# ManUtdMoon/Distributional-Reachability-Policy-Optimization

Measured on AMD Instinct MI355X. Metric: imagined transitions/sec + SAC grad-steps/sec, quadrotor @1/2/4/8 GPU, higher is better.
Workload: dtype fp32

## Files before the change

### distributional-reachability-policy-optimization_amd/csrc/wgrad.hip

```cpp
#include "common.hpp"
#include "ens_nll.hpp"
#include "pack_layout.hpp"

using namespace drpo;

namespace {
constexpr int WG_NW = 4;
constexpr int WG_NT = WG_NW * 64;
constexpr int WG_D = 3;
constexpr int WG_ROWQ = 64;
constexpr int WG_MAXITEMS = 16;
constexpr int WG_SLD = 264;
}

#ifdef DRPO_STAMPS
__device__ unsigned long long g_stamps_wg[1 << 14][8];
#define STAMPG(i)                                                                                 \
  do {                                                                                            \
    __builtin_amdgcn_sched_barrier(0);                                                            \
    unsigned long long _t;                                                                        \
    asm volatile("s_memtime %0\n\ts_waitcnt lgkmcnt(0)" : "=s"(_t)::"memory");                    \
    __builtin_amdgcn_sched_barrier(0);                                                            \
    if (threadIdx.x == 0 && blockIdx.x < (1u << 14)) g_stamps_wg[blockIdx.x][(i)] = _t;           \
  } while (0)
DRPO_API int drpo_debug_stamps_wgrad(unsigned long long* dst, int n) {
  return (int)hipMemcpyFromSymbol(dst, HIP_SYMBOL(g_stamps_wg), sizeof(unsigned long long) * 8 * (size_t)n);
}
DRPO_API int drpo_debug_stamps_wgrad_clear() {
  void* p = nullptr;
  if (hipGetSymbolAddress(&p, HIP_SYMBOL(g_stamps_wg)) != hipSuccess) return 1;
  return (int)hipMemset(p, 0, sizeof(g_stamps_wg));
}
#else
#define STAMPG(i) \
  do {            \
  } while (0)
#endif

struct WgradPlan {
  int to, ti;
  int nto, nti, nch;
  int chunk;
  int va, vb;
  int z2;
  int pk_layer;
  int pk_z0;
  int vf;
  int64_t first_unit;
  int64_t first_tile;
  int64_t slab_off;
};

constexpr int WG_MAXSUMS = 4;

struct WgradArgs {
  int64_t first[WG_MAXITEMS];
  drpo_wgrad_item_t it[WG_MAXITEMS];
  WgradPlan pl[WG_MAXITEMS];
  int64_t units;
  int n;
  int has_red;
  drpo_ens_reduce_t red;
  int nsums;
  drpo_sum_t sums[WG_MAXSUMS];
  int has_adam;
  drpo_wgrad_adam_t adam;
  float* slab;
  unsigned* ctr;
};

typedef const __attribute__((address_space(4))) WgradArgs WgradArgsK;

__device__ __forceinline__ void sums_block(WgradArgsK& a, float* red) {
  for (int q = 0; q < a.nsums; ++q) {
    const auto& S = a.sums[q];
    float v = 0.f;
    for (int j = threadIdx.x; j < S.n; j += WG_NT) v += S.part[j];
    v = block_tree_sum(v, red);
    if (threadIdx.x == 0) *S.out = v;
    __syncthreads();
  }
}

__device__ __forceinline__ void st_sc1(float* p, float v) {
  __hip_atomic_store(p, v, __ATOMIC_RELAXED, __HIP_MEMORY_SCOPE_AGENT);
}
__device__ __forceinline__ float ld_sc1(const float* p) {
  return __hip_atomic_load(const_cast<float*>(p), __ATOMIC_RELAXED, __HIP_MEMORY_SCOPE_AGENT);
}

template <int W, bool VEC>
__device__ __forceinline__ f32x4 frag_load(const float* __restrict__ M, int64_t row, int64_t ld, int c, int ncols) {
  const float* p = M + row * ld + c;
  f32x4 v;
  if constexpr (W == 4 && VEC) {
    v = gload(reinterpret_cast<const f32x4*>(p));
  } else if constexpr (W == 4) {
#pragma unroll
    for (int u = 0; u < 4; ++u) v[u] = gload(c + u < ncols ? p + u : p);
  } else {
    v = f32x4{gload(p), 0.f, 0.f, 0.f};
  }
  return v;
}

template <int TO, int TI>
__device__ __forceinline__ void frag_mma(const f32x4& a, const f32x4& b, f32x4 (&acc)[TO / 16][TI / 16]) {
  constexpr int MA = TO / 16, MB = TI / 16;
  if constexpr (MA == 4 && MB == 4) {
#pragma unroll
    for (int m = 0; m < 4; ++m)
#pragma unroll
      for (int n = 0; n < 4; ++n) acc[m][n] = __builtin_amdgcn_mfma_f32_16x16x4f32(a[m], b[n], acc[m][n], 0, 0, 0);
  } else if constexpr (MA == 4) {
#pragma unroll
    for (int m = 0; m < 4; ++m) acc[m][0] = __builtin_amdgcn_mfma_f32_16x16x4f32(a[m], b[0], acc[m][0], 0, 0, 0);
  } else if constexpr (MB == 4) {
#pragma unroll
    for (int n = 0; n < 4; ++n) acc[0][n] = __builtin_amdgcn_mfma_f32_16x16x4f32(a[0], b[n], acc[0][n], 0, 0, 0);
  } else {
    acc[0][0] = __builtin_amdgcn_mfma_f32_16x16x4f32(a[0], b[0], acc[0][0], 0, 0, 0);
  }
}

template <int TO, int TI>
__device__ __forceinline__ int slab_index(int w, int ol, int il) {
  constexpr int NA = (TO / 16) * (TI / 16), NB = TI / 16;
  int m, rr, G, n, L;
  if constexpr (TO == 64) {
    m = ol & 3; rr = (ol >> 2) & 3; G = ol >> 4;
  } else {
    m = 0; rr = ol & 3; G = ol >> 2;
  }
  if constexpr (TI == 64) {
    n = il & 3; L = il >> 2;
  } else {
    n = 0; L = il;
  }
  return (w * NA + m * NB + n) * WG_SLD + rr * 64 + 16 * G + L;
}

__device__ __forceinline__ float wg_block_sum(float v, float* red) {
  v = wave_sum(v);
  const int lane = threadIdx.x & 63, w = threadIdx.x >> 6;
  __syncthreads();
  if (lane == 0) red[w] = v;
  __syncthreads();
  float s = 0.f;
  if (threadIdx.x == 0)
    for (int i = 0; i < WG_NW; ++i) s += red[i];
  return s;
}

struct WgUnit {
  int zb, ch;
  int o0, i0;
  int dout, din;
  int64_t tile_local;
  int64_t r0, r1;
  bool do_bias;
  bool bias_mine;
  float *gW, *gb;
  int64_t eW, eb;
};

template <int TO, int TI>
__device__ __forceinline__ WgUnit unit_decode(WgradArgsK& a, int q, int64_t u) {
  const auto& I = a.it[q];
  const auto& P = a.pl[q];
  WgUnit U;
  const unsigned uu = (unsigned)u;
  const int it_i = (int)(uu % (unsigned)P.nti);
  unsigned rest = uu / (unsigned)P.nti;
  const int it_o = (int)(rest % (unsigned)P.nto);
  rest /= (unsigned)P.nto;
  U.ch = (int)(rest % (unsigned)P.nch);
  U.zb = (int)(rest / (unsigned)P.nch);
  U.tile_local = ((int64_t)U.zb * P.nto + it_o) * P.nti + it_i;
  U.dout = I.dout;
  U.din = I.din;
  U.o0 = it_o * TO;
  U.i0 = it_i * TI;
  U.r0 = (int64_t)U.ch * P.chunk;
  U.r1 = min(I.rows, U.r0 + P.chunk);
  U.do_bias = it_i == 0;
  U.bias_mine = U.do_bias && (int)threadIdx.x < TO && U.o0 + (int)threadIdx.x < U.dout;
  U.gW = I.gW + (size_t)U.zb * I.gwstride;
  U.gb = I.gb + (size_t)U.zb * I.gbstride;
  U.eW = a.has_adam ? U.gW - a.adam.g : 0;
  U.eb = a.has_adam ? U.gb - a.adam.g : 0;
  return U;
}

template <int TO, int TI, bool VA, bool VB, bool Z2>
__device__ __forceinline__ void wgrad_accumulate(WgradArgsK& a, int q, const WgUnit& U,
                                                 f32x4 (&acc)[TO / 16][TI / 16], f32x4& bsum) {
  constexpr int MA = TO / 16, MB = TI / 16;
  constexpr int WA = TO == 64 ? 4 : 1, WB = TI == 64 ? 4 : 1;
  const auto& I = a.it[q];
  const auto& P = a.pl[q];
  const int lane = threadIdx.x & 63, wave = threadIdx.x >> 6;
  const int g = lane >> 4, l15 = lane & 15;
  const int dout = U.dout, din = U.din;
  const float* __restrict__ dz = I.dz + (size_t)U.zb * I.zstride;
  const float* __restrict__ dz2 = Z2 ? I.dz2 + (size_t)U.zb * I.zstride : nullptr;
  const float* __restrict__ y = I.y + (size_t)U.zb * I.ystride;
  const int64_t r1 = U.r1;
  const bool do_bias = U.do_bias;

  const int ca_raw = U.o0 + (WA == 4 ? 4 * l15 : l15);
  const int cb_raw = U.i0 + (WB == 4 ? 4 * l15 : l15);
  const int ca = ca_raw < dout ? ca_raw : 0, cb = cb_raw < din ? cb_raw : 0;

#pragma unroll
  for (int m = 0; m < MA; ++m)
#pragma unroll
    for (int n = 0; n < MB; ++n) acc[m][n] = f32x4{0.f, 0.f, 0.f, 0.f};
  bsum = f32x4{0.f, 0.f, 0.f, 0.f};

  const int nj = P.chunk / (4 * WG_NW);
  const int64_t rlane = U.r0 + 4 * wave + g;
  auto ld = [&](int j, f32x4& fa, f32x4& fb, f32x4& fa2) {
    const int64_t r = rlane + 16 * (int64_t)j;
    const int64_t rc = r < r1 ? r : r1 - 1;
    fa = frag_load<WA, VA>(dz, rc, dout, ca, dout);
    fb = frag_load<WB, VB>(y, rc, din, cb, din);
    if constexpr (Z2) fa2 = frag_load<WA, VA>(dz2, rc, dout, ca, dout);
  };
  auto use = [&](int j, f32x4 fa, const f32x4& fb, const f32x4& fa2) {
    if constexpr (Z2) fa += fa2;
    if (rlane + 16 * (int64_t)j >= r1) fa = f32x4{0.f, 0.f, 0.f, 0.f};
    frag_mma<TO, TI>(fa, fb, acc);
    if (do_bias) bsum += fa;
  };
  f32x4 ra[WG_D], rb[WG_D], ra2[Z2 ? WG_D : 1];
#pragma unroll
  for (int v = 0; v < WG_D; ++v) ra[v] = rb[v] = f32x4{0.f, 0.f, 0.f, 0.f};
#pragma unroll
  for (int v = 0; v < (Z2 ? WG_D : 1); ++v) ra2[v] = f32x4{0.f, 0.f, 0.f, 0.f};
  const int steps = (nj + WG_D - 1 + WG_D - 1) / WG_D * WG_D;
  STAMPG(6);
  for (int s0 = 0; s0 < steps; s0 += WG_D) {
#pragma unroll
    for (int v = 0; v < WG_D; ++v) {
      ld(s0 + v, ra[v], rb[v], ra2[Z2 ? v : 0]);
      __builtin_amdgcn_sched_barrier(0);
      if (s0 + v >= WG_D - 1)
        use(s0 + v - (WG_D - 1), ra[(v + 1) % WG_D], rb[(v + 1) % WG_D], ra2[Z2 ? (v + 1) % WG_D : 0]);
    }
#ifdef DRPO_STAMPS
    if (s0 == 0) STAMPG(7);
    if (s0 == WG_D) STAMPG(5);
#endif
  }
  STAMPG(1);
}

template <int TI, int W>
__device__ __forceinline__ void run_at(int j, int& ol, int& il) {
  const int f = threadIdx.x + WG_NT * j;
  ol = f / (TI / W);
  il = f % (TI / W) * W;
}
template <int W>
__device__ __forceinline__ void run_load(const float* p, bool in, float* x) {
  if constexpr (W == 4) {
    float t[4] = {0.f, 0.f, 0.f, 0.f};
    if (in) load_row4(p, true, 4, t);
#pragma unroll
    for (int c = 0; c < 4; ++c) x[c] = t[c];
  } else {
    x[0] = in ? *p : 0.f;
  }
}
template <int W>
__device__ __forceinline__ void run_store(float* p, const float* x) {
  if constexpr (W == 4) {
    const float t[4] = {x[0], x[1], x[2], x[3]};
    store_row4(p, true, 4, t);
  } else {
    *p = x[0];
  }
}

template <int E>
struct TileCur {
  float g[E], p[E], m[E], v[E];
  float bg, bp, bm, bv;
};

template <int TO, int TI, int W>
__device__ __forceinline__ void tile_load(WgradArgsK& a, const WgUnit& U, TileCur<TO * TI / WG_NT>& c) {
  constexpr int E = TO * TI / WG_NT;
  const int tid = threadIdx.x;
  const bool adam = a.has_adam;
#pragma unroll
  for (int j = 0; j < E / W; ++j) {
    int ol, il;
    run_at<TI, W>(j, ol, il);
    const int o = U.o0 + ol, i = U.i0 + il;
    const bool in = o < U.dout && i < U.din;
    const int64_t k = (int64_t)o * U.din + i;
    run_load<W>(U.gW + k, in, c.g + W * j);
    if (adam) {
      run_load<W>(a.adam.p + U.eW + k, in, c.p + W * j);
      run_load<W>(a.adam.m + U.eW + k, in, c.m + W * j);
      run_load<W>(a.adam.v + U.eW + k, in, c.v + W * j);
    }
  }
  c.bg = U.bias_mine ? U.gb[U.o0 + tid] : 0.f;
  c.bp = c.bm = c.bv = 0.f;
  if (adam && U.bias_mine) {
    c.bp = a.adam.p[U.eb + U.o0 + tid];
    c.bm = a.adam.m[U.eb + U.o0 + tid];
    c.bv = a.adam.v[U.eb + U.o0 + tid];
  }
}

template <int TO, int TI, int W>
__device__ __forceinline__ void wave_combine(const f32x4 (&acc)[TO / 16][TI / 16], f32x4 bsum, const WgUnit& U,
                                             float* lds, float (&pv)[TO * TI / WG_NT], float& pb) {
  constexpr int MA = TO / 16, MB = TI / 16, NA = MA * MB, E = TO * TI / WG_NT;
  const int tid = threadIdx.x, lane = tid & 63, wave = tid >> 6;
  const int g = lane >> 4, l15 = lane & 15;
  float* R = lds;
#pragma unroll
  for (int m = 0; m < MA; ++m)
#pragma unroll
    for (int n = 0; n < MB; ++n)
#pragma unroll
      for (int rr = 0; rr < 4; ++rr) R[(wave * NA + m * MB + n) * WG_SLD + rr * 64 + lane] = acc[m][n][rr];
  float* Rb = lds + WG_NW * NA * WG_SLD;
  if (U.do_bias) {
#pragma unroll
    for (int c = 0; c < 4; ++c) {
      float s = bsum[c];
      s += __shfl_xor(s, 16, 64);
      s += __shfl_xor(s, 32, 64);
      bsum[c] = s;
    }
    if (g == 0) {
      if constexpr (TO == 64) {
#pragma unroll
        for (int c = 0; c < 4; ++c) Rb[wave * TO + 4 * l15 + c] = bsum[c];
      } else {
        Rb[wave * TO + l15] = bsum[0];
      }
    }
  }
  __syncthreads();
#pragma unroll
  for (int j = 0; j < E / W; ++j) {
    int ol, il;
    run_at<TI, W>(j, ol, il);
#pragma unroll
    for (int c = 0; c < W; ++c) {
      float s = 0.f;
#pragma unroll
      for (int w = 0; w < WG_NW; ++w) s += R[slab_index<TO, TI>(w, ol, il + c)];
      pv[W * j + c] = s;
    }
  }
  pb = 0.f;
  if (U.do_bias && tid < TO) {
#pragma unroll
    for (int w = 0; w < WG_NW; ++w) pb += Rb[w * TO + tid];
  }
}

template <int TO, int TI>
__device__ __forceinline__ bool slab_publish(WgradArgsK& a, int q, const WgUnit& U, const float (&pv)[TO * TI / WG_NT],
                                             float pb, float* red) {
  constexpr int E = TO * TI / WG_NT, SL = TO * TI + TO;
  const auto& P = a.pl[q];
  const int tid = threadIdx.x;
  float* my = a.slab + P.slab_off + (U.tile_local * P.nch + U.ch) * SL;
#pragma unroll
  for (int e = 0; e < E; ++e) st_sc1(my + tid + WG_NT * e, pv[e]);
  if (U.do_bias && tid < TO) st_sc1(my + TO * TI + tid, pb);
  asm volatile("s_waitcnt vmcnt(0)" ::: "memory");
  __syncthreads();
  int& s_last = *reinterpret_cast<int*>(red + 4);
  if (tid == 0) {
    unsigned* c = a.ctr + P.first_tile + U.tile_local;
    const unsigned old = __hip_atomic_fetch_add(c, 1u, __ATOMIC_RELAXED, __HIP_MEMORY_SCOPE_AGENT);
    const int last = old == (unsigned)(P.nch - 1);
    if (last) __hip_atomic_store(c, 0u, __ATOMIC_RELAXED, __HIP_MEMORY_SCOPE_AGENT);
    s_last = last;
  }
  __syncthreads();
  STAMPG(3);
  return s_last;
}

template <int TO, int TI>
__device__ __forceinline__ void slab_sum(WgradArgsK& a, int q, const WgUnit& U, float (&pv)[TO * TI / WG_NT],
                                         float& pb) {
  constexpr int E = TO * TI / WG_NT, SL = TO * TI + TO;
  const auto& P = a.pl[q];
  const int tid = threadIdx.x;
  const float* base = a.slab + P.slab_off + U.tile_local * P.nch * SL;
  const bool bias_lane = U.do_bias && tid < TO;
#pragma unroll
  for (int e = 0; e < E; ++e) pv[e] = 0.f;
  pb = 0.f;
  constexpr int CG = E >= 16 ? 4 : 8;
  for (int c0 = 0; c0 < P.nch; c0 += CG) {
    float t[CG][E], tb[CG];
#pragma unroll
    for (int u = 0; u < CG; ++u) {
      const int c = min(c0 + u, P.nch - 1);
#pragma unroll
      for (int e = 0; e < E; ++e) t[u][e] = ld_sc1(base + c * SL + tid + WG_NT * e);
      tb[u] = bias_lane ? ld_sc1(base + c * SL + TO * TI + tid) : 0.f;
    }
#pragma unroll
    for (int u = 0; u < CG; ++u) {
      if (c0 + u < P.nch) {
#pragma unroll
        for (int e = 0; e < E; ++e) pv[e] += t[u][e];
        pb += tb[u];
      }
    }
  }
}

template <int TO, int TI, int W>
__device__ __forceinline__ void finish_adam(WgradArgsK& a, int q, const WgUnit& U, TileCur<TO * TI / WG_NT>& c,
                                            const float (&pv)[TO * TI / WG_NT], float pb, float* lds) {
  constexpr int E = TO * TI / WG_NT;
  const auto& P = a.pl[q];
  const int tid = threadIdx.x;
  const int dout = U.dout, din = U.din;
  const drpo_pack_map_t* md = P.pk_layer >= 0 ? (const drpo_pack_map_t*)a.adam.map : nullptr;
  const int ncb = pack_frags(dout), nks = pack_frags(din);
  const int64_t mb = md ? pack_member_base(md->poff[P.pk_layer], P.pk_z0 + U.zb, ncb, nks) : 0;
  float* PM = md ? md->P : nullptr;
  float* PTM = md ? md->PT : nullptr;
#pragma unroll
  for (int j = 0; j < E / W; ++j) {
    int ol, il;
    run_at<TI, W>(j, ol, il);
    const int o = U.o0 + ol, i = U.i0 + il;
    if (o >= dout || i >= din) continue;
    const int64_t k = (int64_t)o * din + i;
    bool nz = false;
#pragma unroll
    for (int w = 0; w < W; ++w) {
      const int e = W * j + w;
      adam_step(a.adam, 1.f, c.g[e] + pv[e], c.p[e], c.m[e], c.v[e]);
      nz = nz || c.g[e] != 0.f;
    }
    run_store<W>(a.adam.p + U.eW + k, c.p + W * j);
    run_store<W>(a.adam.m + U.eW + k, c.m + W * j);
    run_store<W>(a.adam.v + U.eW + k, c.v + W * j);
    const float zero[4] = {0.f, 0.f, 0.f, 0.f};
    if (nz) run_store<W>(U.gW + k, zero);
    if (PM) run_store<W>(PM + mb + pack_fwd_index(o, i, nks), c.p + W * j);
    if constexpr (W == 1)
      if (PTM) PTM[mb + pack_tr_index(o, i, ncb)] = c.p[j];
  }
  if constexpr (W == 4) {
    if (PTM) {
      float* T = lds;
      __syncthreads();
#pragma unroll
      for (int j = 0; j < E / 4; ++j) {
        int ol, il;
        run_at<TI, 4>(j, ol, il);
        const bool in = U.o0 + ol < dout && U.i0 + il < din;
#pragma unroll
        for (int w = 0; w < 4; ++w) T[ol * 65 + il + w] = in ? c.p[4 * j + w] : 0.f;
      }
      __syncthreads();
#pragma unroll
      for (int j = 0; j < E / 4; ++j) {
        const int f = tid + WG_NT * j;
        const int il = f >> 4, ol = (f & 15) << 2;
        const int o = U.o0 + ol, i = U.i0 + il;
        if (o >= dout || i >= din) continue;
        float v[4];
#pragma unroll
        for (int w = 0; w < 4; ++w) v[w] = T[(ol + w) * 65 + il];
        run_store<4>(PTM + mb + pack_tr_index(o, i, ncb), v);
      }
    }
  }
  if (U.bias_mine) {
    adam_step(a.adam, 1.f, c.bg + pb, c.bp, c.bm, c.bv);
    a.adam.p[U.eb + U.o0 + tid] = c.bp;
    a.adam.m[U.eb + U.o0 + tid] = c.bm;
    a.adam.v[U.eb + U.o0 + tid] = c.bv;
    if (c.bg != 0.f) U.gb[U.o0 + tid] = 0.f;
  }
}

template <int TO, int TI, int W>
__device__ __forceinline__ void finish_grad(WgradArgsK& a, int q, const WgUnit& U, const TileCur<TO * TI / WG_NT>& c,
                                            const float (&pv)[TO * TI / WG_NT], float pb, float* red) {
  constexpr int E = TO * TI / WG_NT;
  const auto& I = a.it[q];
  const int tid = threadIdx.x;
  float sq = 0.f;
#pragma unroll
  for (int j = 0; j < E / W; ++j) {
    int ol, il;
    run_at<TI, W>(j, ol, il);
    const int o = U.o0 + ol, i = U.i0 + il;
    if (o >= U.dout || i >= U.din) continue;
    float v[W];
#pragma unroll
    for (int w = 0; w < W; ++w) {
      v[w] = c.g[W * j + w] + pv[W * j + w];
      sq = fmaf(v[w], v[w], sq);
    }
    run_store<W>(U.gW + (size_t)o * U.din + i, v);
  }
  if (U.bias_mine) {
    const float v = c.bg + pb;
    U.gb[U.o0 + tid] = v;
    sq = fmaf(v, v, sq);
  }
  if (I.sq) {
    const float s = wg_block_sum(sq, red);
    if (tid == 0) I.sq[I.sq_off + U.tile_local] = s;
  }
}

template <int TO, int TI, int W>
__device__ __forceinline__ void wgrad_tile(WgradArgsK& a, int q, const WgUnit& U, const f32x4 (&acc)[TO / 16][TI / 16],
                                           const f32x4& bsum, float* lds) {
  constexpr int E = TO * TI / WG_NT;
  const auto& P = a.pl[q];
  float* red = lds + WG_NW * (TO / 16) * (TI / 16) * WG_SLD + WG_NW * TO;
  TileCur<E> cur;
  if (P.nch == 1) tile_load<TO, TI, W>(a, U, cur);
  float pv[E], pb;
  wave_combine<TO, TI, W>(acc, bsum, U, lds, pv, pb);
  STAMPG(2);
  if (P.nch > 1) {
    if (!slab_publish<TO, TI>(a, q, U, pv, pb, red)) return;
    tile_load<TO, TI, W>(a, U, cur);
    slab_sum<TO, TI>(a, q, U, pv, pb);
  }
  if (a.has_adam) finish_adam<TO, TI, W>(a, q, U, cur, pv, pb, lds);
  else finish_grad<TO, TI, W>(a, q, U, cur, pv, pb, red);
  STAMPG(4);
}

template <int TO, int TI>
__device__ __forceinline__ void wgrad_unit(WgradArgsK& a, int q, int64_t u, float* lds) {
  const auto& P = a.pl[q];
  const WgUnit U = unit_decode<TO, TI>(a, q, u);
  f32x4 acc[TO / 16][TI / 16], bsum;
  switch ((P.z2 ? 4 : 0) | (P.va ? 2 : 0) | (P.vb ? 1 : 0)) {
    case 0: wgrad_accumulate<TO, TI, false, false, false>(a, q, U, acc, bsum); break;
    case 1: wgrad_accumulate<TO, TI, false, true, false>(a, q, U, acc, bsum); break;
    case 2: wgrad_accumulate<TO, TI, true, false, false>(a, q, U, acc, bsum); break;
    case 3: wgrad_accumulate<TO, TI, true, true, false>(a, q, U, acc, bsum); break;
    case 4: wgrad_accumulate<TO, TI, false, false, true>(a, q, U, acc, bsum); break;
    case 5: wgrad_accumulate<TO, TI, false, true, true>(a, q, U, acc, bsum); break;
    case 6: wgrad_accumulate<TO, TI, true, false, true>(a, q, U, acc, bsum); break;
    default: wgrad_accumulate<TO, TI, true, true, true>(a, q, U, acc, bsum); break;
  }
  if constexpr (TO == 64 && TI == 64) {
    if (P.vf) return wgrad_tile<TO, TI, 4>(a, q, U, acc, bsum, lds);
  }
  wgrad_tile<TO, TI, 1>(a, q, U, acc, bsum, lds);
}

__global__ __launch_bounds__(WG_NT, 2) void mlp_wgrad_kernel(WgradArgs args) {
  extern __shared__ __attribute__((aligned(16))) float wsm[];
  WgradArgsK& a = *(const __attribute__((address_space(4))) WgradArgs*)__builtin_amdgcn_kernarg_segment_ptr();
  (void)args;
  STAMPG(0);
  const int64_t bid = xcd_block().x;
  if (bid >= a.units) {
    if (a.has_red && bid == a.units) {
      typedef const __attribute__((address_space(4))) drpo_wgrad_adam_t AdamK;
      ens_loss_reduce_block(a.red, a.has_adam ? &a.adam : (AdamK*)nullptr);
    }
    else if (a.nsums) sums_block(a, wsm);
    return;
  }
  const int q = block_item<WG_MAXITEMS>(a, bid);
  const auto& P = a.pl[q];
  const int64_t u = bid - P.first_unit;
  if (P.to == 64 && P.ti == 64) wgrad_unit<64, 64>(a, q, u, wsm);
  else if (P.to == 64) wgrad_unit<64, 16>(a, q, u, wsm);
  else if (P.ti == 64) wgrad_unit<16, 64>(a, q, u, wsm);
  else wgrad_unit<16, 16>(a, q, u, wsm);
}

static_assert(sizeof(WgradArgs) <= 4096, "weight-gradient kernarg");

static size_t wgrad_lds() { return sizeof(float) * ((size_t)WG_NW * 16 * WG_SLD + WG_NW * 64 + 8); }

namespace {

struct Plan {
  WgradArgs a;
  int64_t tiles;
  int64_t slab;
};

int wg_cus() {
  static int cus = [] {
    int dev = 0, n = 0;
    if (hipGetDevice(&dev) != hipSuccess || hipDeviceGetAttribute(&n, hipDeviceAttributeMultiprocessorCount, dev) !=
                                                 hipSuccess || n <= 0)
      n = 256;
    return n;
  }();
  return cus;
}

int kg_cost(int to, int ti) { return to == 64 && ti == 64 ? 16 : (to == 64 || ti == 64 ? 6 : 3); }

int plan(const drpo_wgrad_item_t* items, int n, const drpo_ens_reduce_t* red, Plan& p) {
  WgradArgs& a = p.a;
  a = WgradArgs{};
  int m = 0;
  struct Shape { int to, ti, nto, nti; int64_t rows, nb; };
  Shape sh[WG_MAXITEMS];
  for (int k = 0; k < n; ++k) {
    const drpo_wgrad_item_t& I = items[k];
    DRPO_REQUIRE(I.dz && I.y && I.gW && I.gb && I.dout >= 1 && I.din >= 1 && I.rows >= 0 && I.nbatch >= 1,
                 "drpo_mlp_wgrad: bad item %d", k);
    DRPO_REQUIRE(!I.sq || I.sq_off >= 0, "drpo_mlp_wgrad: item %d sq_off", k);
    for (int j = 0; j < k; ++j)
      DRPO_REQUIRE(items[j].gW != I.gW, "drpo_mlp_wgrad: items %d and %d write the same gradient", j, k);
    if (I.rows == 0) continue;
    a.it[m] = I;
    Shape& s = sh[m];
    s.to = I.dout <= 16 ? 16 : 64;
    s.ti = I.din <= 16 ? 16 : 64;
    s.nto = (I.dout + s.to - 1) / s.to;
    s.nti = (I.din + s.ti - 1) / s.ti;
    s.rows = I.rows;
    s.nb = I.nbatch;
    ++m;
  }
  a.n = m;
  const int64_t slots = 2 * (int64_t)wg_cus();
  auto units_for = [&](double per, int* nch, int* chunk) {
    int64_t tot = 0;
    for (int k = 0; k < m; ++k) {
      const Shape& s = sh[k];
      const double rows_per = per * 16.0 / kg_cost(s.to, s.ti);
      int64_t c = (int64_t)((double)s.rows / (rows_per > 1 ? rows_per : 1) + 0.5);
      c = c < 1 ? 1 : c;
      int64_t ck = (s.rows + c - 1) / c;
      ck = (ck + WG_ROWQ - 1) / WG_ROWQ * WG_ROWQ;
      c = (s.rows + ck - 1) / ck;
      nch[k] = (int)c;
      chunk[k] = (int)ck;
      tot += c * s.nto * s.nti * s.nb;
    }
    return tot;
  };
  double total = 0;
  for (int k = 0; k < m; ++k)
    total += (double)sh[k].nb * sh[k].nto * sh[k].nti * ((sh[k].rows + 15) / 16) * kg_cost(sh[k].to, sh[k].ti);
  int nch[WG_MAXITEMS], chunk[WG_MAXITEMS];
  double per = total / (double)slots;
  if (per < 1) per = 1;
  for (int it = 0; it < 64 && units_for(per, nch, chunk) > slots; ++it) per *= 1.08;
  int64_t unit = 0, tile = 0, slab = 0;
  for (int k = 0; k < m; ++k) {
    const Shape& s = sh[k];
    WgradPlan& P = a.pl[k];
    const drpo_wgrad_item_t& I = a.it[k];
    P.to = s.to; P.ti = s.ti; P.nto = s.nto; P.nti = s.nti; P.nch = nch[k]; P.chunk = chunk[k];
    P.va = (I.dout & 3) == 0 && ((uintptr_t)I.dz & 15) == 0 && ((uintptr_t)I.dz2 & 15) == 0 && (I.zstride & 3) == 0;
    P.z2 = I.dz2 != nullptr;
    P.vb = (I.din & 3) == 0 && ((uintptr_t)I.y & 15) == 0 && (I.ystride & 3) == 0;
    P.vf = s.to == 64 && s.ti == 64 && (I.din & 3) == 0 && ((uintptr_t)I.gW & 15) == 0 && (I.gwstride & 3) == 0;
    P.first_unit = unit;
    P.first_tile = tile;
    P.slab_off = slab;
    const int64_t ntile = (int64_t)s.nto * s.nti * s.nb;
    unit += ntile * P.nch;
    tile += ntile;
    if (P.nch > 1) slab += ntile * P.nch * ((int64_t)s.to * s.ti + s.to);
  }
  for (int k = 0; k < WG_MAXITEMS; ++k) a.first[k] = k < m ? a.pl[k].first_unit : INT64_MAX;
  a.units = unit;
  p.tiles = tile;
  p.slab = slab;
  if (red) {
    a.has_red = 1;
    a.red = *red;
  }
  return DRPO_OK;
}

size_t ctr_bytes(const Plan& p) { return (size_t)((p.tiles * 4 + 255) / 256 * 256); }
size_t ws_bytes(const Plan& p) { return ctr_bytes(p) + sizeof(float) * (size_t)p.slab; }

int match_pack_layer(const drpo_pack_map_t& mh, const drpo_wgrad_item_t& I, const float* g, int k, WgradPlan& P) {
  const int64_t off = I.gW - g;
  for (int l = 0; l < mh.nlayers && l < 16; ++l) {
    const int64_t per = (int64_t)mh.din[l] * mh.dout[l], rel = off - mh.off[l];
    if (mh.din[l] != I.din || mh.dout[l] != I.dout || rel < 0 || rel % per != 0) continue;
    const int64_t z0 = rel / per;
    if (z0 + I.nbatch > mh.nbatch[l] || (I.nbatch > 1 && I.gwstride != per)) continue;
    DRPO_REQUIRE(P.pk_layer < 0, "drpo_mlp_wgrad_adam: item %d matches layers %d and %d of the pack map", k,
                 P.pk_layer, l);
    P.pk_layer = l;
    P.pk_z0 = (int)z0;
  }
  DRPO_REQUIRE(P.pk_layer >= 0, "drpo_mlp_wgrad_adam: item %d is not a matrix of the pack map", k);
  return DRPO_OK;
}

}

DRPO_API int drpo_mlp_wgrad_tiles(const drpo_wgrad_item_t* I) {
  if (!I || I->dout < 1 || I->din < 1 || I->nbatch < 1) return 0;
  const int to = I->dout <= 16 ? 16 : 64, ti = I->din <= 16 ? 16 : 64;
  return ((I->dout + to - 1) / to) * ((I->din + ti - 1) / ti) * I->nbatch;
}

DRPO_API size_t drpo_mlp_wgrad_workspace_size(const drpo_wgrad_item_t* items, int n) {
  if (n < 0 || n > WG_MAXITEMS || (n > 0 && !items)) return 0;
  Plan p;
  if (plan(items, n, nullptr, p) != DRPO_OK) return 0;
  return ws_bytes(p);
}

DRPO_API int drpo_mlp_wgrad(const drpo_wgrad_item_t* items, int n, void* workspace, size_t workspace_bytes,
                            drpo_stream_t stream) {
  return drpo_mlp_wgrad_reduce(items, n, nullptr, workspace, workspace_bytes, stream);
}

static int wgrad_launch(const drpo_wgrad_item_t* items, int n, const drpo_ens_reduce_t* red, const drpo_sum_t* sums,
                        int nsums, void* workspace, size_t workspace_bytes, hipStream_t stream,
                        const drpo_wgrad_adam_t* adam = nullptr);

DRPO_API int drpo_mlp_wgrad_adam(const drpo_wgrad_item_t* items, int n, const drpo_ens_reduce_t* red,
                                 const drpo_wgrad_adam_t* adam, void* workspace, size_t workspace_bytes,
                                 drpo_stream_t stream_) {
  if (const int e = red ? ens_reduce_check("drpo_mlp_wgrad_adam", red) : DRPO_OK) return e;
  DRPO_REQUIRE(adam && adam->g && adam->p && adam->m && adam->v && adam->bc2_sqrt > 0.f &&
                   (!adam->map == !adam->map_host),
               "drpo_mlp_wgrad_adam: bad Adam descriptor (g, p, m, v; map with its host copy)");
  for (int k = 0; k < n; ++k)
    DRPO_REQUIRE(!items[k].sq, "drpo_mlp_wgrad_adam: item %d asks for clip partials (no clip in the fused step)", k);
  return wgrad_launch(items, n, red, nullptr, 0, workspace, workspace_bytes, (hipStream_t)stream_, adam);
}

DRPO_API int drpo_mlp_wgrad_reduce(const drpo_wgrad_item_t* items, int n, const drpo_ens_reduce_t* red,
                                   void* workspace, size_t workspace_bytes, drpo_stream_t stream_) {
  if (const int e = red ? ens_reduce_check("drpo_mlp_wgrad_reduce", red) : DRPO_OK) return e;
  return wgrad_launch(items, n, red, nullptr, 0, workspace, workspace_bytes, (hipStream_t)stream_);
}

DRPO_API int drpo_mlp_wgrad_sums(const drpo_wgrad_item_t* items, int n, const drpo_sum_t* sums, int nsums,
                                 void* workspace, size_t workspace_bytes, drpo_stream_t stream_) {
  DRPO_REQUIRE(nsums >= 0 && nsums <= WG_MAXSUMS && (nsums == 0 || sums), "drpo_mlp_wgrad_sums: 0..%d sums",
               WG_MAXSUMS);
  for (int q = 0; q < nsums; ++q)
    DRPO_REQUIRE(sums[q].n >= 0 && sums[q].out && (sums[q].n == 0 || sums[q].part), "drpo_mlp_wgrad_sums: sum %d", q);
  return wgrad_launch(items, n, nullptr, sums, nsums, workspace, workspace_bytes, (hipStream_t)stream_);
}

static int wgrad_launch(const drpo_wgrad_item_t* items, int n, const drpo_ens_reduce_t* red, const drpo_sum_t* sums,
                        int nsums, void* workspace, size_t workspace_bytes, hipStream_t stream,
                        const drpo_wgrad_adam_t* adam) {
  DRPO_REQUIRE(n >= 0 && n <= WG_MAXITEMS && (n == 0 || items), "drpo_mlp_wgrad: at most %d items", WG_MAXITEMS);
  static Plan p;
  const int rc = plan(items, n, red, p);
  if (rc != DRPO_OK) return rc;
  const size_t need = ws_bytes(p);
  DRPO_REQUIRE(workspace_bytes >= need && (need == 0 || workspace),
               "drpo_mlp_wgrad: workspace %zu bytes < %zu (drpo_mlp_wgrad_workspace_size)", workspace_bytes, need);
  p.a.ctr = (unsigned*)workspace;
  p.a.slab = (float*)((char*)workspace + ctr_bytes(p));
  p.a.nsums = nsums;
  for (int q = 0; q < nsums; ++q) p.a.sums[q] = sums[q];
  p.a.has_adam = adam != nullptr;
  if (adam) {
    p.a.adam = *adam;
    const drpo_pack_map_t* mh = (const drpo_pack_map_t*)adam->map_host;
    for (int k = 0; k < p.a.n; ++k) {
      p.a.pl[k].pk_layer = -1;
      p.a.pl[k].pk_z0 = 0;
      if (!mh) continue;
      if (const int e = match_pack_layer(*mh, p.a.it[k], adam->g, k, p.a.pl[k])) return e;
    }
    const bool al = ((uintptr_t)adam->p & 15) == 0 && ((uintptr_t)adam->m & 15) == 0 &&
                    ((uintptr_t)adam->v & 15) == 0 && ((uintptr_t)adam->g & 15) == 0 &&
                    (!mh || (((uintptr_t)mh->P & 15) == 0 && ((uintptr_t)mh->PT & 15) == 0));
    for (int k = 0; k < p.a.n; ++k) p.a.pl[k].vf = p.a.pl[k].vf && al && ((p.a.it[k].gW - adam->g) & 3) == 0;
  }
  const int64_t blocks = p.a.units + (red ? 1 : 0) + (nsums ? 1 : 0);
  if (blocks == 0) return DRPO_OK;
  mlp_wgrad_kernel<<<(unsigned)blocks, WG_NT, wgrad_lds(), stream>>>(p.a);
  DRPO_LAUNCH_CHECK("mlp_wgrad");
  return DRPO_OK;
}
```

Before: 194.7 million.

## Slim wgrad kernarg layout, use magic-number division and branchless item lookup

Replaces the per-item kernel argument struct with compact head/tail records so the accumulate phase reads only the fields it needs. Unit decode uses precomputed magic multipliers instead of integer division, and the item index comes from a branchless scalar compare-and-add chain. Tile variant flags are packed into one word, 32-bit indices replace 64-bit ones, and the slab-sum chunk group for small tiles grows from 8 to 16. The aim is to cut fixed per-block setup cost in a kernel launched with many short blocks. In exchange it adds an int32 range limit on units and tiles and relies on the magic-division math being exact.

```diff
diff --git a/distributional-reachability-policy-optimization_amd/csrc/wgrad.hip b/distributional-reachability-policy-optimization_amd/csrc/wgrad.hip
--- a/distributional-reachability-policy-optimization_amd/csrc/wgrad.hip
+++ b/distributional-reachability-policy-optimization_amd/csrc/wgrad.hip
@@ -51,13 +51,38 @@
   int64_t slab_off;
 };
 
+enum : int { WG_VB = 1, WG_VA = 2, WG_Z2 = 4, WG_TI64 = 8, WG_TO64 = 16, WG_VF = 32 };
+
+struct WgradHead {
+  const float *dz, *y, *dz2;
+  int64_t zstride, ystride;
+  int64_t rows;
+  int dout, din;
+  int first_unit;
+  int chunk;
+  int nti, nto, nch;
+  unsigned m_ti, m_to, m_ch;
+  int shifts;
+  int variant;
+};
+
+struct WgradTail {
+  float *gW, *gb;
+  int64_t gwstride, gbstride;
+  float* sq;
+  int64_t slab_off;
+  int first_tile;
+  int sq_off;
+  int pk_layer, pk_z0;
+};
+
 constexpr int WG_MAXSUMS = 4;
 
 struct WgradArgs {
-  int64_t first[WG_MAXITEMS];
-  drpo_wgrad_item_t it[WG_MAXITEMS];
-  WgradPlan pl[WG_MAXITEMS];
-  int64_t units;
+  int first[WG_MAXITEMS];
+  WgradHead hd[WG_MAXITEMS];
+  WgradTail tl[WG_MAXITEMS];
+  int units;
   int n;
   int has_red;
   drpo_ens_reduce_t red;
@@ -156,55 +181,70 @@
   int zb, ch;
   int o0, i0;
   int dout, din;
+  int nj;
+  int nch;
+  int variant;
+  int64_t r0, r1;
+  const float *dz, *dz2, *y;
+  bool do_bias;
   int64_t tile_local;
-  int64_t r0, r1;
-  bool do_bias;
   bool bias_mine;
   float *gW, *gb;
   int64_t eW, eb;
 };
 
-template <int TO, int TI>
-__device__ __forceinline__ WgUnit unit_decode(WgradArgsK& a, int q, int64_t u) {
-  const auto& I = a.it[q];
-  const auto& P = a.pl[q];
+__device__ __forceinline__ unsigned magic_div(unsigned x, unsigned m, int s) {
+  return (unsigned)(((uint64_t)x * m) >> s);
+}
+
+__device__ __forceinline__ WgUnit unit_head(WgradArgsK& a, int q, unsigned bid) {
+  const auto& H = a.hd[q];
   WgUnit U;
-  const unsigned uu = (unsigned)u;
-  const int it_i = (int)(uu % (unsigned)P.nti);
-  unsigned rest = uu / (unsigned)P.nti;
-  const int it_o = (int)(rest % (unsigned)P.nto);
-  rest /= (unsigned)P.nto;
-  U.ch = (int)(rest % (unsigned)P.nch);
-  U.zb = (int)(rest / (unsigned)P.nch);
-  U.tile_local = ((int64_t)U.zb * P.nto + it_o) * P.nti + it_i;
-  U.dout = I.dout;
-  U.din = I.din;
-  U.o0 = it_o * TO;
-  U.i0 = it_i * TI;
-  U.r0 = (int64_t)U.ch * P.chunk;
-  U.r1 = min(I.rows, U.r0 + P.chunk);
+  const unsigned uu = bid - (unsigned)H.first_unit;
+  const int sh = H.shifts;
+  unsigned rest = magic_div(uu, H.m_ti, sh & 63);
+  const int it_i = (int)(uu - rest * (unsigned)H.nti);
+  const unsigned rest2 = magic_div(rest, H.m_to, (sh >> 8) & 63);
+  const int it_o = (int)(rest - rest2 * (unsigned)H.nto);
+  U.zb = (int)magic_div(rest2, H.m_ch, (sh >> 16) & 63);
+  U.ch = (int)(rest2 - (unsigned)U.zb * (unsigned)H.nch);
+  U.variant = H.variant;
+  U.tile_local = ((int64_t)U.zb * H.nto + it_o) * H.nti + it_i;
+  U.dout = H.dout;
+  U.din = H.din;
+  U.o0 = it_o << (U.variant & WG_TO64 ? 6 : 4);
+  U.i0 = it_i << (U.variant & WG_TI64 ? 6 : 4);
+  U.nj = H.chunk / (4 * WG_NW);
+  U.nch = H.nch;
+  U.r0 = (int64_t)U.ch * H.chunk;
+  U.r1 = min(H.rows, U.r0 + H.chunk);
   U.do_bias = it_i == 0;
+  U.dz = H.dz + (size_t)U.zb * H.zstride;
+  U.dz2 = reinterpret_cast<const float*>(reinterpret_cast<uintptr_t>(H.dz2) + sizeof(float) * (size_t)U.zb * H.zstride);
+  U.y = H.y + (size_t)U.zb * H.ystride;
+  return U;
+}
+
+template <int TO>
+__device__ __forceinline__ void unit_tail(WgradArgsK& a, int q, WgUnit& U) {
+  const auto& T = a.tl[q];
   U.bias_mine = U.do_bias && (int)threadIdx.x < TO && U.o0 + (int)threadIdx.x < U.dout;
-  U.gW = I.gW + (size_t)U.zb * I.gwstride;
-  U.gb = I.gb + (size_t)U.zb * I.gbstride;
+  U.gW = T.gW + (size_t)U.zb * T.gwstride;
+  U.gb = T.gb + (size_t)U.zb * T.gbstride;
   U.eW = a.has_adam ? U.gW - a.adam.g : 0;
   U.eb = a.has_adam ? U.gb - a.adam.g : 0;
-  return U;
 }
 
 template <int TO, int TI, bool VA, bool VB, bool Z2>
-__device__ __forceinline__ void wgrad_accumulate(WgradArgsK& a, int q, const WgUnit& U,
-                                                 f32x4 (&acc)[TO / 16][TI / 16], f32x4& bsum) {
+__device__ __forceinline__ void wgrad_accumulate(const WgUnit& U, f32x4 (&acc)[TO / 16][TI / 16], f32x4& bsum) {
   constexpr int MA = TO / 16, MB = TI / 16;
   constexpr int WA = TO == 64 ? 4 : 1, WB = TI == 64 ? 4 : 1;
-  const auto& I = a.it[q];
-  const auto& P = a.pl[q];
   const int lane = threadIdx.x & 63, wave = threadIdx.x >> 6;
   const int g = lane >> 4, l15 = lane & 15;
   const int dout = U.dout, din = U.din;
-  const float* __restrict__ dz = I.dz + (size_t)U.zb * I.zstride;
-  const float* __restrict__ dz2 = Z2 ? I.dz2 + (size_t)U.zb * I.zstride : nullptr;
-  const float* __restrict__ y = I.y + (size_t)U.zb * I.ystride;
+  const float* __restrict__ dz = U.dz;
+  const float* __restrict__ dz2 = Z2 ? U.dz2 : nullptr;
+  const float* __restrict__ y = U.y;
   const int64_t r1 = U.r1;
   const bool do_bias = U.do_bias;
 
@@ -218,7 +258,7 @@
     for (int n = 0; n < MB; ++n) acc[m][n] = f32x4{0.f, 0.f, 0.f, 0.f};
   bsum = f32x4{0.f, 0.f, 0.f, 0.f};
 
-  const int nj = P.chunk / (4 * WG_NW);
+  const int nj = U.nj;
   const int64_t rlane = U.r0 + 4 * wave + g;
   auto ld = [&](int j, f32x4& fa, f32x4& fb, f32x4& fa2) {
     const int64_t r = rlane + 16 * (int64_t)j;
@@ -276,10 +316,9 @@
 template <int W>
 __device__ __forceinline__ void run_store(float* p, const float* x) {
   if constexpr (W == 4) {
-    const float t[4] = {x[0], x[1], x[2], x[3]};
-    store_row4(p, true, 4, t);
+    gstore(reinterpret_cast<f32x4*>(p), f32x4{x[0], x[1], x[2], x[3]});
   } else {
-    *p = x[0];
+    gstore(p, x[0]);
   }
 }
 
@@ -372,9 +411,9 @@
 __device__ __forceinline__ bool slab_publish(WgradArgsK& a, int q, const WgUnit& U, const float (&pv)[TO * TI / WG_NT],
                                              float pb, float* red) {
   constexpr int E = TO * TI / WG_NT, SL = TO * TI + TO;
-  const auto& P = a.pl[q];
+  const auto& T = a.tl[q];
   const int tid = threadIdx.x;
-  float* my = a.slab + P.slab_off + (U.tile_local * P.nch + U.ch) * SL;
+  float* my = a.slab + T.slab_off + (U.tile_local * U.nch + U.ch) * SL;
 #pragma unroll
   for (int e = 0; e < E; ++e) st_sc1(my + tid + WG_NT * e, pv[e]);
   if (U.do_bias && tid < TO) st_sc1(my + TO * TI + tid, pb);
@@ -382,9 +421,9 @@
   __syncthreads();
   int& s_last = *reinterpret_cast<int*>(red + 4);
   if (tid == 0) {
-    unsigned* c = a.ctr + P.first_tile + U.tile_local;
+    unsigned* c = a.ctr + T.first_tile + U.tile_local;
     const unsigned old = __hip_atomic_fetch_add(c, 1u, __ATOMIC_RELAXED, __HIP_MEMORY_SCOPE_AGENT);
-    const int last = old == (unsigned)(P.nch - 1);
+    const int last = old == (unsigned)(U.nch - 1);
     if (last) __hip_atomic_store(c, 0u, __ATOMIC_RELAXED, __HIP_MEMORY_SCOPE_AGENT);
     s_last = last;
   }
@@ -397,26 +436,26 @@
 __device__ __forceinline__ void slab_sum(WgradArgsK& a, int q, const WgUnit& U, float (&pv)[TO * TI / WG_NT],
                                          float& pb) {
   constexpr int E = TO * TI / WG_NT, SL = TO * TI + TO;
-  const auto& P = a.pl[q];
+  const int nch = U.nch;
   const int tid = threadIdx.x;
-  const float* base = a.slab + P.slab_off + U.tile_local * P.nch * SL;
+  const float* base = a.slab + a.tl[q].slab_off + U.tile_local * nch * SL;
   const bool bias_lane = U.do_bias && tid < TO;
 #pragma unroll
   for (int e = 0; e < E; ++e) pv[e] = 0.f;
   pb = 0.f;
-  constexpr int CG = E >= 16 ? 4 : 8;
-  for (int c0 = 0; c0 < P.nch; c0 += CG) {
+  constexpr int CG = E >= 16 ? 4 : 16;
+  for (int c0 = 0; c0 < nch; c0 += CG) {
     float t[CG][E], tb[CG];
 #pragma unroll
     for (int u = 0; u < CG; ++u) {
-      const int c = min(c0 + u, P.nch - 1);
+      const int c = min(c0 + u, nch - 1);
 #pragma unroll
       for (int e = 0; e < E; ++e) t[u][e] = ld_sc1(base + c * SL + tid + WG_NT * e);
       tb[u] = bias_lane ? ld_sc1(base + c * SL + TO * TI + tid) : 0.f;
     }
 #pragma unroll
     for (int u = 0; u < CG; ++u) {
-      if (c0 + u < P.nch) {
+      if (c0 + u < nch) {
 #pragma unroll
         for (int e = 0; e < E; ++e) pv[e] += t[u][e];
         pb += tb[u];
@@ -429,12 +468,12 @@
 __device__ __forceinline__ void finish_adam(WgradArgsK& a, int q, const WgUnit& U, TileCur<TO * TI / WG_NT>& c,
                                             const float (&pv)[TO * TI / WG_NT], float pb, float* lds) {
   constexpr int E = TO * TI / WG_NT;
-  const auto& P = a.pl[q];
+  const auto& T = a.tl[q];
   const int tid = threadIdx.x;
   const int dout = U.dout, din = U.din;
-  const drpo_pack_map_t* md = P.pk_layer >= 0 ? (const drpo_pack_map_t*)a.adam.map : nullptr;
+  const drpo_pack_map_t* md = T.pk_layer >= 0 ? (const drpo_pack_map_t*)a.adam.map : nullptr;
   const int ncb = pack_frags(dout), nks = pack_frags(din);
-  const int64_t mb = md ? pack_member_base(md->poff[P.pk_layer], P.pk_z0 + U.zb, ncb, nks) : 0;
+  const int64_t mb = md ? pack_member_base(md->poff[T.pk_layer], T.pk_z0 + U.zb, ncb, nks) : 0;
   float* PM = md ? md->P : nullptr;
   float* PTM = md ? md->PT : nullptr;
 #pragma unroll
@@ -458,7 +497,7 @@
     if (nz) run_store<W>(U.gW + k, zero);
     if (PM) run_store<W>(PM + mb + pack_fwd_index(o, i, nks), c.p + W * j);
     if constexpr (W == 1)
-      if (PTM) PTM[mb + pack_tr_index(o, i, ncb)] = c.p[j];
+      if (PTM) gstore(PTM + mb + pack_tr_index(o, i, ncb), c.p[j]);
   }
   if constexpr (W == 4) {
     if (PTM) {
@@ -499,7 +538,7 @@
 __device__ __forceinline__ void finish_grad(WgradArgsK& a, int q, const WgUnit& U, const TileCur<TO * TI / WG_NT>& c,
                                             const float (&pv)[TO * TI / WG_NT], float pb, float* red) {
   constexpr int E = TO * TI / WG_NT;
-  const auto& I = a.it[q];
+  const auto& I = a.tl[q];
   const int tid = threadIdx.x;
   float sq = 0.f;
 #pragma unroll
@@ -531,14 +570,13 @@
 __device__ __forceinline__ void wgrad_tile(WgradArgsK& a, int q, const WgUnit& U, const f32x4 (&acc)[TO / 16][TI / 16],
                                            const f32x4& bsum, float* lds) {
   constexpr int E = TO * TI / WG_NT;
-  const auto& P = a.pl[q];
   float* red = lds + WG_NW * (TO / 16) * (TI / 16) * WG_SLD + WG_NW * TO;
   TileCur<E> cur;
-  if (P.nch == 1) tile_load<TO, TI, W>(a, U, cur);
+  if (U.nch == 1) tile_load<TO, TI, W>(a, U, cur);
   float pv[E], pb;
   wave_combine<TO, TI, W>(acc, bsum, U, lds, pv, pb);
   STAMPG(2);
-  if (P.nch > 1) {
+  if (U.nch > 1) {
     if (!slab_publish<TO, TI>(a, q, U, pv, pb, red)) return;
     tile_load<TO, TI, W>(a, U, cur);
     slab_sum<TO, TI>(a, q, U, pv, pb);
@@ -549,24 +587,29 @@
 }
 
 template <int TO, int TI>
-__device__ __forceinline__ void wgrad_unit(WgradArgsK& a, int q, int64_t u, float* lds) {
-  const auto& P = a.pl[q];
-  const WgUnit U = unit_decode<TO, TI>(a, q, u);
+__device__ __forceinline__ void wgrad_unit(WgradArgsK& a, int q, WgUnit& U, float* lds) {
   f32x4 acc[TO / 16][TI / 16], bsum;
-  switch ((P.z2 ? 4 : 0) | (P.va ? 2 : 0) | (P.vb ? 1 : 0)) {
-    case 0: wgrad_accumulate<TO, TI, false, false, false>(a, q, U, acc, bsum); break;
-    case 1: wgrad_accumulate<TO, TI, false, true, false>(a, q, U, acc, bsum); break;
-    case 2: wgrad_accumulate<TO, TI, true, false, false>(a, q, U, acc, bsum); break;
-    case 3: wgrad_accumulate<TO, TI, true, true, false>(a, q, U, acc, bsum); break;
-    case 4: wgrad_accumulate<TO, TI, false, false, true>(a, q, U, acc, bsum); break;
-    case 5: wgrad_accumulate<TO, TI, false, true, true>(a, q, U, acc, bsum); break;
-    case 6: wgrad_accumulate<TO, TI, true, false, true>(a, q, U, acc, bsum); break;
-    default: wgrad_accumulate<TO, TI, true, true, true>(a, q, U, acc, bsum); break;
-  }
+  switch (U.variant & (WG_Z2 | WG_VA | WG_VB)) {
+    case 0: wgrad_accumulate<TO, TI, false, false, false>(U, acc, bsum); break;
+    case 1: wgrad_accumulate<TO, TI, false, true, false>(U, acc, bsum); break;
+    case 2: wgrad_accumulate<TO, TI, true, false, false>(U, acc, bsum); break;
+    case 3: wgrad_accumulate<TO, TI, true, true, false>(U, acc, bsum); break;
+    case 4: wgrad_accumulate<TO, TI, false, false, true>(U, acc, bsum); break;
+    case 5: wgrad_accumulate<TO, TI, false, true, true>(U, acc, bsum); break;
+    case 6: wgrad_accumulate<TO, TI, true, false, true>(U, acc, bsum); break;
+    default: wgrad_accumulate<TO, TI, true, true, true>(U, acc, bsum); break;
+  }
+  unit_tail<TO>(a, q, U);
   if constexpr (TO == 64 && TI == 64) {
-    if (P.vf) return wgrad_tile<TO, TI, 4>(a, q, U, acc, bsum, lds);
+    if (U.variant & WG_VF) return wgrad_tile<TO, TI, 4>(a, q, U, acc, bsum, lds);
   }
   wgrad_tile<TO, TI, 1>(a, q, U, acc, bsum, lds);
+}
+
+__device__ __forceinline__ unsigned xcd_block_1d() {
+  const unsigned nb = gridDim.x, bid = blockIdx.x;
+  const unsigned q = nb >> 3, r = nb & 7, k = bid & 7;
+  return k * q + (k < r ? k : r) + (bid >> 3);
 }
 
 __global__ __launch_bounds__(WG_NT, 2) void mlp_wgrad_kernel(WgradArgs args) {
@@ -574,8 +617,8 @@
   WgradArgsK& a = *(const __attribute__((address_space(4))) WgradArgs*)__builtin_amdgcn_kernarg_segment_ptr();
   (void)args;
   STAMPG(0);
-  const int64_t bid = xcd_block().x;
-  if (bid >= a.units) {
+  const int bid = (int)xcd_block_1d();
+  if (__builtin_expect(bid >= a.units, 0)) {
     if (a.has_red && bid == a.units) {
       typedef const __attribute__((address_space(4))) drpo_wgrad_adam_t AdamK;
       ens_loss_reduce_block(a.red, a.has_adam ? &a.adam : (AdamK*)nullptr);
@@ -583,13 +626,16 @@
     else if (a.nsums) sums_block(a, wsm);
     return;
   }
-  const int q = block_item<WG_MAXITEMS>(a, bid);
-  const auto& P = a.pl[q];
-  const int64_t u = bid - P.first_unit;
-  if (P.to == 64 && P.ti == 64) wgrad_unit<64, 64>(a, q, u, wsm);
-  else if (P.to == 64) wgrad_unit<64, 16>(a, q, u, wsm);
-  else if (P.ti == 64) wgrad_unit<16, 64>(a, q, u, wsm);
-  else wgrad_unit<16, 16>(a, q, u, wsm);
+  int q = -1;
+#pragma unroll
+  for (int i = 0; i < WG_MAXITEMS; ++i)
+    asm("s_cmp_ge_i32 %1, %2\n\ts_addc_u32 %0, %0, 0" : "+s"(q) : "s"(bid), "s"(a.first[i]) : "scc");
+  WgUnit U = unit_head(a, q, (unsigned)bid);
+  const int shape = U.variant & (WG_TO64 | WG_TI64);
+  if (shape == (WG_TO64 | WG_TI64)) wgrad_unit<64, 64>(a, q, U, wsm);
+  else if (shape == WG_TO64) wgrad_unit<64, 16>(a, q, U, wsm);
+  else if (shape == WG_TI64) wgrad_unit<16, 64>(a, q, U, wsm);
+  else wgrad_unit<16, 16>(a, q, U, wsm);
 }
 
 static_assert(sizeof(WgradArgs) <= 4096, "weight-gradient kernarg");
@@ -598,11 +644,65 @@
 
 namespace {
 
+struct PlanHost {
+  drpo_wgrad_item_t it[WG_MAXITEMS];
+  WgradPlan pl[WG_MAXITEMS];
+  int64_t units;
+  int n;
+  int has_red;
+  drpo_ens_reduce_t red;
+};
+
 struct Plan {
-  WgradArgs a;
+  PlanHost a;
+  WgradArgs dev;
   int64_t tiles;
   int64_t slab;
 };
+
+void magic_of(int d, unsigned& m, int& s) {
+  int L = 0;
+  while (((int64_t)1 << L) < d) ++L;
+  s = 31 + L;
+  m = (unsigned)((((uint64_t)1 << s) + (uint64_t)d - 1) / (uint64_t)d);
+}
+
+void device_args(Plan& p) {
+  const PlanHost& h = p.a;
+  WgradArgs& d = p.dev;
+  d = WgradArgs{};
+  for (int k = 0; k < WG_MAXITEMS; ++k) d.first[k] = k < h.n ? (int)h.pl[k].first_unit : INT32_MAX;
+  for (int k = 0; k < h.n; ++k) {
+    const drpo_wgrad_item_t& I = h.it[k];
+    const WgradPlan& P = h.pl[k];
+    WgradHead& H = d.hd[k];
+    H.dz = I.dz; H.y = I.y; H.dz2 = I.dz2;
+    H.zstride = I.zstride; H.ystride = I.ystride;
+    H.rows = I.rows;
+    H.dout = I.dout; H.din = I.din;
+    H.first_unit = (int)P.first_unit;
+    H.chunk = P.chunk;
+    H.nti = P.nti; H.nto = P.nto; H.nch = P.nch;
+    int s_ti, s_to, s_ch;
+    magic_of(P.nti, H.m_ti, s_ti);
+    magic_of(P.nto, H.m_to, s_to);
+    magic_of(P.nch, H.m_ch, s_ch);
+    H.shifts = s_ti | s_to << 8 | s_ch << 16;
+    H.variant = (P.vb ? WG_VB : 0) | (P.va ? WG_VA : 0) | (P.z2 ? WG_Z2 : 0) | (P.ti == 64 ? WG_TI64 : 0) |
+                (P.to == 64 ? WG_TO64 : 0) | (P.vf ? WG_VF : 0);
+    WgradTail& T = d.tl[k];
+    T.gW = I.gW; T.gb = I.gb;
+    T.gwstride = I.gwstride; T.gbstride = I.gbstride;
+    T.sq = I.sq; T.sq_off = I.sq_off;
+    T.slab_off = P.slab_off;
+    T.first_tile = (int)P.first_tile;
+    T.pk_layer = P.pk_layer; T.pk_z0 = P.pk_z0;
+  }
+  d.units = (int)h.units;
+  d.n = h.n;
+  d.has_red = h.has_red;
+  d.red = h.red;
+}
 
 int wg_cus() {
   static int cus = [] {
@@ -618,8 +718,8 @@
 int kg_cost(int to, int ti) { return to == 64 && ti == 64 ? 16 : (to == 64 || ti == 64 ? 6 : 3); }
 
 int plan(const drpo_wgrad_item_t* items, int n, const drpo_ens_reduce_t* red, Plan& p) {
-  WgradArgs& a = p.a;
-  a = WgradArgs{};
+  PlanHost& a = p.a;
+  a = PlanHost{};
   int m = 0;
   struct Shape { int to, ti, nto, nti; int64_t rows, nb; };
   Shape sh[WG_MAXITEMS];
@@ -684,7 +784,6 @@
     tile += ntile;
     if (P.nch > 1) slab += ntile * P.nch * ((int64_t)s.to * s.ti + s.to);
   }
-  for (int k = 0; k < WG_MAXITEMS; ++k) a.first[k] = k < m ? a.pl[k].first_unit : INT64_MAX;
   a.units = unit;
   p.tiles = tile;
   p.slab = slab;
@@ -775,13 +874,9 @@
   const size_t need = ws_bytes(p);
   DRPO_REQUIRE(workspace_bytes >= need && (need == 0 || workspace),
                "drpo_mlp_wgrad: workspace %zu bytes < %zu (drpo_mlp_wgrad_workspace_size)", workspace_bytes, need);
-  p.a.ctr = (unsigned*)workspace;
-  p.a.slab = (float*)((char*)workspace + ctr_bytes(p));
-  p.a.nsums = nsums;
-  for (int q = 0; q < nsums; ++q) p.a.sums[q] = sums[q];
-  p.a.has_adam = adam != nullptr;
+  DRPO_REQUIRE(p.a.units < INT32_MAX - 2 && p.tiles < INT32_MAX, "drpo_mlp_wgrad: %lld units (< 2^31)",
+               (long long)p.a.units);
   if (adam) {
-    p.a.adam = *adam;
     const drpo_pack_map_t* mh = (const drpo_pack_map_t*)adam->map_host;
     for (int k = 0; k < p.a.n; ++k) {
       p.a.pl[k].pk_layer = -1;
@@ -796,7 +891,14 @@
   }
   const int64_t blocks = p.a.units + (red ? 1 : 0) + (nsums ? 1 : 0);
   if (blocks == 0) return DRPO_OK;
-  mlp_wgrad_kernel<<<(unsigned)blocks, WG_NT, wgrad_lds(), stream>>>(p.a);
+  device_args(p);
+  p.dev.ctr = (unsigned*)workspace;
+  p.dev.slab = (float*)((char*)workspace + ctr_bytes(p));
+  p.dev.nsums = nsums;
+  for (int q = 0; q < nsums; ++q) p.dev.sums[q] = sums[q];
+  p.dev.has_adam = adam != nullptr;
+  if (adam) p.dev.adam = *adam;
+  mlp_wgrad_kernel<<<(unsigned)blocks, WG_NT, wgrad_lds(), stream>>>(p.dev);
   DRPO_LAUNCH_CHECK("mlp_wgrad");
   return DRPO_OK;
 }
diff --git a/profiles/wgrad_fixed_cost/record_parent_digests.py b/profiles/wgrad_fixed_cost/record_parent_digests.py
--- /dev/null
+++ b/profiles/wgrad_fixed_cost/record_parent_digests.py
@@ -0,0 +1,27 @@
+import json
+import os
+import sys
+
+ROOT = os.path.dirname(os.path.dirname(os.path.dirname(os.path.abspath(__file__))))
+sys.path.insert(0, ROOT)
+sys.path.insert(0, os.path.join(ROOT, 'tests'))
+
+
+def main():
+    import test_gpu_wgrad_fixed as t
+    from drpo_amd import _lib
+    out = sys.argv[1] if len(sys.argv) > 1 else t.GOLDEN
+    dig = {}
+    for rows in t.ROWS:
+        for c in t.all_cases(rows):
+            t.check_float64(*c)
+            dig[t.case_key(*c)] = t.digests(*c)
+    rec = {'cus': t.device_cus(), 'library_digest': _lib.build_digest(), 'cases': len(dig), 'digests': dig}
+    with open(out, 'w') as f:
+        json.dump(rec, f, indent=0, sort_keys=True)
+        f.write('\n')
+    print(f'{len(dig)} cases, {rec["cus"]} CUs -> {out}')
+
+
+if __name__ == '__main__':
+    main()
diff --git a/profiles/wgrad_fixed_cost/row_sweep.py b/profiles/wgrad_fixed_cost/row_sweep.py
--- /dev/null
+++ b/profiles/wgrad_fixed_cost/row_sweep.py
@@ -0,0 +1,46 @@
+import argparse
+import json
+import os
+import sys
+
+import numpy as np
+
+ROOT = os.path.dirname(os.path.dirname(os.path.dirname(os.path.abspath(__file__))))
+sys.path.insert(0, ROOT)
+sys.path.insert(0, os.path.join(ROOT, 'profiles'))
+
+ROWS = [256, 512, 1024, 2048, 4096, 8192, 16384, 32768, 65536]
+
+
+def main():
+    import wgrad_probe as wp
+    ap = argparse.ArgumentParser()
+    ap.add_argument('--reps', type=int, default=200)
+    ap.add_argument('--runs', type=int, default=5)
+    args = ap.parse_args()
+
+    def med(shapes, rows):
+        items = wp.make(shapes, rows)
+        t = [wp.time_launch(items, rows, reps=args.reps)[0] for _ in range(args.runs)]
+        return float(np.median(t)), float(min(t))
+
+    out = {'lib': os.environ.get('DRPO_LIB_OVERRIDE', 'product'), 'rows': ROWS, 'critic_us': [], 'critic_min_us': []}
+    for rows in ROWS:
+        m, lo = med(wp.CRITIC, rows)
+        out['critic_us'].append(round(m, 3))
+        out['critic_min_us'].append(round(lo, 3))
+    k, t0 = np.polyfit(np.array(ROWS, float), np.array(out['critic_us']), 1)
+    out['t0_us'] = round(float(t0), 3)
+    out['k_us_per_1024_rows'] = round(float(k) * 1024, 4)
+    k_lo, t0_lo = np.polyfit(np.array(ROWS[:5], float), np.array(out['critic_us'][:5]), 1)
+    out['t0_us_rows_le_4096'] = round(float(t0_lo), 3)
+    out['k_us_per_1024_rows_le_4096'] = round(float(k_lo) * 1024, 4)
+    for name, shapes in (('critic', wp.CRITIC), ('actor', wp.ACTOR), ('mult', wp.MULT), ('256x256', [(256, 256)]),
+                         ('256x14', [(256, wp.SA)]), ('1x256', [(1, 256)])):
+        m, lo = med(shapes, 4096)
+        out[name + '_4096_us'] = [round(m, 3), round(lo, 3)]
+    print(json.dumps(out))
+
+
+if __name__ == '__main__':
+    main()
```

Measured after the change: 194.3 million. About the same (-0.2%).
